# zbackup/zbackup

Measured on AMD Instinct MI355X. Metric: rolling-hash chunking GiB/s (device-resident), higher is better.
Workload: dtype u8; 1 GPU; C2: 1 x 8 GiB seeded random stream, device-resident, W=65536; stream_bytes_per_gpu=8589934592, chunk_max_size=65536, parallelism=replicas x1 (independent streams), chunk_ids=rolling hash

## Files before the change

### zbackup_amd/csrc/zc_device.h

```cpp
#pragma once

#include <hip/hip_runtime.h>
#include <stdint.h>

#include <mutex>
#include <string>

#include "../../include/zchunk.h"

struct zc_bundle_file;
struct zc_bundle_layout;
struct zc_gc_input;
struct zc_gc_output;

namespace zc {

constexpr int ZC_SPAN = 1024;
constexpr int ZC_TPB = 256;
#ifndef ZC_SCAN_TPB_CFG
#define ZC_SCAN_TPB_CFG 512
#endif
#ifndef ZC_LSPAN_CFG
#define ZC_LSPAN_CFG 4096
#endif
// ... 100 lines not shown
__host__ __device__ inline uint32_t chk_bucket(uint64_t key, uint32_t bits) {
  return (uint32_t)((key * 0x9E3779B97F4A7C15ull) >> (64 - bits));
}
__host__ __device__ inline uint32_t chk_match(uint2 v, uint32_t c) {
  const uint32_t s0 = v.x & 0xFFFFu, s1 = v.x >> 16, s2 = v.y & 0xFFFFu, s3 = v.y >> 16;
  if (s0 == c || s1 == c || s2 == c || s3 == c) return 1;
  return (s0 == 0 || s1 == 0 || s2 == 0 || s3 == 0) ? 0 : 2;
}
inline uint32_t chk_bits_for(size_t keys) {
  uint32_t b = 10;
  while (((size_t)4 << b) < 16 * keys) ++b;
  return b;
}
__host__ __device__ inline uint32_t bloom_lo(uint32_t g) {
  return (1u << (g & 31u)) | (1u << ((g >> 5) & 31u)) | (1u << ((g >> 10) & 31u));
}
__host__ __device__ inline uint32_t bloom_hi(uint32_t g) {
  return (1u << ((g >> 15) & 31u)) | (1u << ((g >> 20) & 31u)) | (1u << ((g >> 25) & 31u));
}

struct Run {
  uint64_t start, end;
};

struct Cand {
  uint64_t p;
  uint32_t ref;
  uint32_t pad;
};

enum { CNT_POOL = 0, CNT_OVERFLOW = 1, CNT_CAND = 2, CNT_RUNS = 3, CNT_FOVF = 4, CNT_ANCLESS = 5, CNT_CLASS = 6,
       CNT_PAIRS = 7, CNT_SPAIRS = 8, CNT_LAST = 9 };

hipError_t launch_scan(const uint8_t* data, uint64_t n, int32_t anchor_lo, uint64_t* blk, PoolOut po,
                       unsigned long long* counters, hipStream_t s);
hipError_t launch_scan_tiles(const uint8_t* data, uint64_t n, uint64_t tile0, uint64_t ntiles, int32_t anchor_lo,
                             uint64_t* blk, PoolOut po, unsigned long long* counters, hipStream_t s,
                             GridKeysOut gko = GridKeysOut{nullptr, nullptr, 0, 0}, hipEvent_t start = nullptr,
                             hipEvent_t stop = nullptr, uint32_t max_wgs = 0, uint32_t* tiles_per_wave = nullptr);
inline uint32_t scan_key_lshift_or_none(uint32_t W, bool& ok) {
  ok = W >= (uint32_t)ZC_LSPAN && W % ZC_LSPAN == 0 && ((64u * ZC_LSPAN) % W) == 0;
  uint32_t l = 0;
  while (ok && ((uint32_t)ZC_LSPAN << l) < W) ++l;
  return l;
}
hipError_t launch_scan_tail(const uint8_t* data, uint64_t n, int32_t anchor_lo, uint64_t* blk, PoolOut po,
                            unsigned long long* counters, hipStream_t s, hipEvent_t start = nullptr,
                            hipEvent_t stop = nullptr);

hipError_t launch_anchor_rescan(const uint8_t* data, uint64_t n, int32_t anchor_lo, const uint32_t* tiles,
                                const uint32_t* sbase, uint32_t ntiles, int pass, uint32_t* base, uint32_t* cnt,
                                uint32_t* srel, uint32_t* sg, hipStream_t s);

struct EpochIndex {
  uint64_t* start;
  uint64_t* vis;
  uint8_t* dead;
  uint64_t* key;
  uint32_t* cg;
  uint64_t* cfp;
  uint32_t* anc;
  uint32_t* cls;
  uint64_t* ckeys;
  uint32_t cbits;
  uint64_t* tab;
  uint32_t tbits;
  uint32_t* gfilt;
  uint32_t* ancless;
  unsigned long long* counters;
  uint2* pairs;
  const uint8_t* gsha;
  uint64_t n_gsha;
// ... 278 lines not shown
```

### zbackup_amd/csrc/zc_engine.cpp

```cpp
#include <hip/hip_runtime.h>
#include <stdint.h>
#include <stdio.h>
#include <stdlib.h>
#include <string.h>
#include <unistd.h>
#include <emmintrin.h>

#include <algorithm>
#include <atomic>
#include <chrono>
#include <exception>
#include <condition_variable>
#include <functional>
#include <iterator>
#include <mutex>
#include <string>
#include <thread>
#include <unordered_map>
#include <vector>

#include "../../include/zchunk.h"
#include "zc_device.h"
#include "zc_lzo_dec.h"

// ... 391 lines not shown
  uint64_t scan_out_keys = 0;
  uint32_t scan_out_tpw = 0;
  uint32_t test_scan_wgs = 0;
  HostBuf<unsigned long long> h_co_hc;
  HostBuf<Cand> h_hist_cand;
  HostBuf<uint32_t> h_cls;
  HostBuf<Run> h_runs;
  size_t nrec_done = 0;
  size_t rec_head = 0;
  mutable std::recursive_mutex mu;
  zc_stats stats{};

  LzoScratch* lzo = nullptr;
  DevBuf<uint8_t> lzo_in, lzo_out;
  AesScratch* aes = nullptr;
  GcScratch* gc = nullptr;
  MetaScratch* meta = nullptr;
  RangeScratch* range = nullptr;
  IndexScratch* index = nullptr;
  ResolveScratch* rs = nullptr;
  XzScratch* xz = nullptr;
  XzEncScratch* xzenc = nullptr;

  DevBuf<uint64_t> hm_key, hm_fp, hm_rkey;
  DevBuf<uint32_t> hm_anc, hm_g, gidx;
  DevBuf<uint64_t> blk, ftile_off;
  DevBuf<uint32_t> ftile_cnt;
  DevBuf<uint32_t> dbase, dcnt;
  DevBuf<uint32_t> prel, pg, srel, sg;
  DevBuf<uint32_t> otiles, obase;
  DevBuf<unsigned long long> counters;
  DevBuf<unsigned long long> scnt;
  bool scnt_dirty = true;
  DevBuf<uint8_t> gsha;
  HostBuf<uint2> h_pairs;
  HostBuf<uint8_t> h_gsha;
  HostBuf<uint64_t> h_hmkey;
  HostBuf<uint32_t> h_hmanc;
  DevBuf<uint64_t> c_start, c_key, c_fp, c_vis;
  DevBuf<uint32_t> c_anc, c_g;
  DevBuf<uint8_t> c_dead;
  DevBuf<uint64_t> ckeys;
  DevBuf<uint32_t> c_cls;
  DevBuf<uint64_t> tab;
  DevBuf<uint32_t> gfilt;
  DevBuf<Cand> cand;
  DevBuf<uint64_t> va, vb, dout;
  DevBuf<uint32_t> vlen;
  DevBuf<uint8_t> vok, sha_out;
  DevBuf<uint32_t> f32, fbits, fbits17;
  DevBuf<uint64_t> fwt_off;
  DevBuf<uint32_t> fwt_cnt;
  DevBuf<Run> runs;
  DevBuf<uint32_t> ancless;
  DevBuf<uint2> cpairs;
  HostBuf<unsigned long long> h_cnt;
  HostBuf<unsigned long long> h_scnt;
  HostBuf<uint64_t> h_pre;
  HostBuf<uint64_t> h_key;
  HostBuf<uint64_t> h_ra, h_rb, h_rout;
};

namespace {

struct DeviceGuard {
  int prev = -1;
// ... 224 lines not shown
    scan_keys_ = kok && !windowed_ && indexable_ && n_ >= W_ && n_ / W_ < 0xFFFFFFF0ull;
    if (scan_keys_) {
      c_.c_key.ensure(n_ / W_ + 2);
      c_.h_key.ensure(n_ / W_ + 2);
    }
    scan_setup();
  }
  void set_avail(uint64_t n) {
    n_ = n;
    c_.stats.bytes = n;
  }
  void clear_tables() {
    if (c_.tables_clean || (!c_.ckeys.p && !c_.tab.p)) return;
    if (c_.ckeys.cap % 2 || c_.tab.cap % 2 || c_.gfilt.cap % 4) return;
    HCK(launch_tables_clear(c_.ckeys.p, c_.ckeys.p ? c_.ckeys.cap : 0, c_.tab.p, c_.tab.p ? c_.tab.cap : 0,
                            c_.gfilt.p, c_.gfilt.p ? c_.gfilt.cap : 0, c_.stream));
    c_.tables_clean = true;
  }
  hipEvent_t scan_end_event() const { return (c_.flags & ZC_FLAG_TIMING) ? c_.ev1 : c_.ev_idx; }
  void scan_upto(uint64_t m, bool last = false) {
    const uint64_t t1 = std::min(m, n_) / ZC_STILE;
    if (t1 > tiles_done_) {
      hipEvent_t start = nullptr;
      if (!scan_open_) {
        if (c_.flags & ZC_FLAG_TIMING) start = c_.ev0;
        scan_open_ = true;
      }
      scnt_pending_ = true;
      const GridKeysOut gko = scan_keys_ ? GridKeysOut{c_.c_key.p, c_.h_key.p, pow257(W_), key_lshift_}
                                         : GridKeysOut{nullptr, nullptr, 0, 0};
      hipEvent_t stop = last ? scan_end_event() : nullptr;
      uint32_t tpw = 0;
      HCK(launch_scan_tiles(d_, n_, tiles_done_, t1 - tiles_done_, anchor_lo_, blk_v(), pool_out(), c_.scnt.p,
                            c_.stream, gko, start, stop, c_.test_scan_wgs, &tpw));
      scan_tpw_ = std::max(scan_tpw_, tpw);
      scan_end_recorded_ = stop != nullptr;
      tiles_done_ = t1;
    }
  }
  uint64_t scanned_end() const { return tiles_done_ * ZC_STILE; }

  void run_segment(uint64_t lim) {
    const auto t0 = Clock::now();
    scan_upto(lim);
    lim = std::min(lim, scanned_end());
    if (lim <= x0()) return;
    scan_finish();
    lim_ = lim;
    final_ = false;
    while (epoch()) {
    }
    if (!scan_checked_) {
      sync(c_);
      scan_check();
    }
    finalize_records();
    c_.stats.segments++;
    c_.stats.total_ms += ms_since(t0);
  }

  void run_final() {
    const auto t0 = Clock::now();
    if (n_ > 0) {
      const bool tail = n_ % ZC_STILE != 0;
      scan_upto(n_, !tail);
      if (tail) {
        hipEvent_t start = nullptr;
// ... 299 lines not shown
  std::vector<ACand>& acands_ = c_.res_acands;
  std::vector<ACand>& hcands_ = c_.res_hcands;

  struct FBatch {
    std::vector<uint64_t> pos, h;
    std::vector<int64_t> vref;
    std::vector<uint8_t> vok;
    std::vector<uint8_t> sha;
    std::vector<uint8_t> has_sha;
    size_t cur = 0;
  } fb_;

  struct Piece {
    size_t rec;
    uint64_t a, b;
  };
  std::vector<Piece> need_digest_;

  void scan_setup() {
    const uint64_t nwt = wave_tiles(cap_);
    if (nwt * wcap_ >= ZC_SIDE_POOL) throw ZcError{ZC_ERR_NOMEM, "stream too large for the anchor pool"};
    c_.blk.ensure((cap_ + ZC_SPAN - 1) / ZC_SPAN);
    c_.dbase.ensure(nwt);
    c_.dcnt.ensure(nwt);
    c_.prel.ensure(nwt * wcap_);
    c_.pg.ensure(nwt * wcap_);
    c_.srel.ensure(1);
    c_.sg.ensure(1);
    if (!c_.counters.p) {
      c_.counters.ensure(CNT_LAST);
      HCK(hipMemsetAsync(c_.counters.p, 0, CNT_LAST * sizeof(unsigned long long), c_.stream));
    }
    c_.h_cnt.ensure(CNT_LAST);
    c_.scnt.ensure(2);
    c_.h_scnt.ensure(CNT_LAST);
    if (c_.scnt_dirty) {
      HCK(hipMemsetAsync(c_.scnt.p, 0, 2 * sizeof(unsigned long long), c_.stream));
      c_.scnt_dirty = false;
    }
  }

  void scan_finish() {
    meta_from_scan_ = scan_open_;
    if (scan_open_) {
      if (!scan_end_recorded_) HCK(hipEventRecord(scan_end_event(), c_.stream));
      side_wait_ = scan_end_event();
      scan_end_ev_ = side_wait_;
    }
    scan_end_recorded_ = false;
    scan_checked_ = false;
  }
  void scan_counters_readback() {
    if (!scnt_pending_) return;
    scnt_pending_ = false;
    d2h(c_, c_.h_scnt.p, c_.scnt.p, 2);
    HCK(hipMemsetAsync(c_.scnt.p, 0, 2 * sizeof(unsigned long long), c_.stream));
  }

  bool scan_check() {
    if (scan_checked_) return false;
    if (scnt_pending_) {
      scan_counters_readback();
      sync(c_);
    }
    scan_checked_ = true;
    if ((c_.flags & ZC_FLAG_TIMING) && scan_open_) {
      float ms = 0;
      HCK(hipEventElapsedTime(&ms, c_.ev0, c_.ev1));
      c_.stats.scan_ms += ms;
    }
    scan_open_ = false;
    const uint64_t wt_lo = chk_wt_, wt_hi = nwt_done();
    chk_wt_ = wt_hi;
    const uint64_t found = c_.h_scnt[CNT_POOL];
    npool_ += found;
    c_.stats.anchors += found;
    if (c_.h_scnt[CNT_OVERFLOW] && wt_hi > wt_lo) {
      const uint64_t nw = wt_hi - wt_lo;
      std::vector<uint32_t> cnt(nw), tiles, sbase;
      d2h(c_, cnt.data(), dcnt_v() + wt_lo, nw);
      sync(c_);
      for (uint64_t t = 0; t < nw; ++t)
        if (cnt[t] == 0xFFFFFFFFu) tiles.push_back((uint32_t)(wt_lo + t));
      const uint32_t nt = (uint32_t)tiles.size();
      if (!nt) return false;
      c_.otiles.ensure(nt);
      c_.obase.ensure(nt);
      h2d(c_, c_.otiles.p, tiles.data(), nt);
      HCK(launch_anchor_rescan(d_, n_, anchor_lo_, c_.otiles.p, nullptr, nt, 0, dbase_v(), dcnt_v(), nullptr, nullptr,
                               c_.stream));
      std::vector<uint32_t> cnt2(nw);
      d2h(c_, cnt2.data(), dcnt_v() + wt_lo, nw);
      sync(c_);
      uint64_t total = 0;
      for (uint32_t t : tiles) {
        sbase.push_back((uint32_t)(side_used_ + total));
        total += cnt2[t - wt_lo];
      }
      if (side_used_ + total >= ZC_SIDE_POOL) throw ZcError{ZC_ERR_NOMEM, "anchor side pool too large"};
      npool_ += total;
      c_.stats.anchors += total;
      c_.srel.grow_keep(side_used_ + total, side_used_, c_.stream);
      c_.sg.grow_keep(side_used_ + total, side_used_, c_.stream);
      h2d(c_, c_.obase.p, sbase.data(), nt);
      HCK(launch_anchor_rescan(d_, n_, anchor_lo_, c_.otiles.p, c_.obase.p, nt, 1, dbase_v(), dcnt_v(), c_.srel.p,
                               c_.sg.p, c_.stream));
      side_used_ += total;
      return true;
    }
    return false;
  }
  bool scan_checked_ = true;
  bool scnt_pending_ = false;
  bool meta_from_scan_ = false;
  hipEvent_t side_wait_ = nullptr;
  hipEvent_t scan_end_ev_ = nullptr;

  bool epoch() {
    if (!scan_checked_ && c_.stats.epochs > 0) {
      sync(c_);
      scan_check();
    }
    c_.stats.epochs++;
    r_e_ = s_;
    ks_ = 0;
    grec_ = grec_valid_ = false;
    const uint64_t xs = x0();
    h_end_ = hspan_ ? std::min<uint64_t>(lim_, xs + hspan_) : lim_;
    nspec_ = (n_ >= r_e_ + 2ull * W_) ? (uint32_t)((n_ - r_e_ - 2ull * W_) / W_ + 1) : 0;
    if (h_end_ < n_) {
      const uint64_t kh = h_end_ - r_e_ >= 2ull * W_ ? (h_end_ - r_e_) / W_ - 1 : 0;
      nspec_ = (uint32_t)std::min<uint64_t>(nspec_, kh);
    }
    const uint32_t nsref = indexable_ ? nspec_ : 0;
    nref_ = nconf_ + nsref;
    dead_.assign(nref_, 0);
    ndead_ = 0;
    cls_.clear();
    acands_.clear();
    hcands_.clear();
    runs_.clear();
    fmap_.clear();
    fmemo_valid_ = false;
    fb_ = FBatch{};
    fb_next_ = kInf;
    has_f_ = false;
// ... 31 lines not shown
        c_.c_dead.ensure(nref_);
        c_.ancless.ensure(nref_);
        c_.h_key.ensure(nsref);
        if (nconf_) {
          h2d(c_, c_.c_start.p, cstart_.data(), nconf_);
          h2d(c_, c_.c_key.p, ckey_.data(), nconf_);
          h2d(c_, c_.c_fp.p, cfp_.data(), nconf_);
          h2d(c_, c_.c_anc.p, canc_.data(), nconf_);
          h2d(c_, c_.c_g.p, cg_.data(), nconf_);
          HCK(hipMemsetAsync(c_.c_vis.p, 0, nconf_ * sizeof(uint64_t), c_.stream));
          HCK(hipMemsetAsync(c_.c_dead.p, 0, nconf_, c_.stream));
        }
        tabs_new |= c_.ckeys.ensure(1u << tbits);
        if (tabs_new) {
          c_.tables_clean = false;
          c_.paths |= ZC_PATH_TABLES_REALLOCATED;
        }
        c_.c_cls.ensure(nref_);
        c_.cpairs.ensure(nref_);
        ix = EpochIndex{c_.c_start.p, c_.c_vis.p, c_.c_dead.p, c_.c_key.p,
                        c_.c_g.p,     c_.c_fp.p,  c_.c_anc.p,  c_.c_cls.p,
                        c_.ckeys.p,   tbits,      anchors ? c_.tab.p : nullptr, tbits,
                        c_.gfilt.p,   c_.ancless.p, c_.counters.p, c_.cpairs.p,
                        pre_sha_n_ ? c_.h_gsha.p : nullptr, pre_sha_n_, nsref ? c_.h_key.p : nullptr};
        ix.key_from = key_from;
        ix.tables_clean = c_.tables_clean;
        c_.tables_clean = false;
        if (key_from) c_.paths |= ZC_PATH_SCAN_KEYS;
        c_.paths |= epoch_index_fused(ix, nconf_, nsref) ? ZC_PATH_FUSED_INSERT : ZC_PATH_TABLES_CLEARED_BY_EPOCH;
        if (scnt_pending_) {
          ix.scnt = c_.scnt.p;
          ix.h_scnt = c_.h_scnt.p;
          scnt_pending_ = false;
        }
        grec_valid_ = false;
        grec_ = !windowed_ && indexable_ && nsref >= kGridRecordsMin;
        grec_ev_ = key_from == nsref && scan_end_ev_ ? scan_end_ev_ : c_.ev_grec;
        HCK(launch_epoch_index(d_, n_, blk_v(), av(), r_e_, nconf_, nsref, W_, pow257(W_), ix, c_.stream,
                               grec_ && grec_ev_ == c_.ev_grec ? c_.ev_grec : nullptr));
        dev_r_e_ = r_e_;
        dev_nconf_ = nconf_;
        dev_nspec_ = nsref;
        dev_valid_ = true;
      } else {
        HCK(hipMemsetAsync(c_.counters.p, 0, CNT_LAST * sizeof(unsigned long long), c_.stream));
        scan_counters_readback();
      }
      const uint64_t* tab = nref_ && anchors ? c_.tab.p : nullptr;
      const bool early_join = spec_ && nref_ && pre_sha_n_;
      if (early_join) HCK(launch_class_sha(nullptr, pre_sha_n_, n_, W_, ix, nref_, c_.stream));
      if (anchors)
        HCK(launch_probe(d_, av(), pwt0(), pwt1() - pwt0(), tab, tbits, c_.gfilt.p, c_.c_anc.p, c_.c_cls.p,
                         c_.c_vis.p, c_.c_dead.p, r_, h_end_, W_, ht, r_e_, nconf_, nsref, c_.cand.p, c_.cand.cap, c_.counters.p,
                         c_.stream));
      if (side_wait_) {
        HCK(hipStreamWaitEvent(c_.copy_stream, side_wait_, 0));
        side_wait_ = nullptr;
      }
      predict_tail();
      HCK(hipEventRecord(c_.ev_copy, c_.copy_stream));
      if (nsref >= kParallelRecordsMin) SpinTeam::get().arm();
      const bool first = !scan_checked_ && meta_from_scan_;
      HCK(launch_counters_out(c_.counters.p, c_.h_cnt.p, c_.stream));
      hipEvent_t batch_ev = c_.ev_batch;
      if (first && (c_.flags & ZC_FLAG_TIMING)) batch_ev = c_.ev_meta;
      HCK(hipEventRecord(batch_ev, c_.stream));
// ... 3136 lines not shown
```

### zbackup_amd/csrc/zc_kernels.hip

```cpp
#include <hip/hip_ext.h>
#include <hip/hip_runtime.h>
#include <stdint.h>

#include <algorithm>

#include "zc_device.h"

namespace zc {

namespace {

constexpr uint64_t kGolden = 0x9E3779B97F4A7C15ull;
typedef unsigned v2u32 __attribute__((ext_vector_type(2)));

#define ZC_URGENT() __builtin_amdgcn_s_setprio(3)

__host__ __device__ inline uint64_t pow257_dev(uint64_t e) {
  uint64_t r = 1, b = 257;
  while (e) {
    if (e & 1) r *= b;
    b *= b;
    e >>= 1;
  }
  return r;
// ... 278 lines not shown
    });
  }
  return tot;
}

typedef __attribute__((address_space(3))) void lds_void_t;
typedef __attribute__((address_space(1))) const void gbl_void_t;

template <int N>
__device__ __forceinline__ void wait_vmcnt() {
  static_assert(N >= 0 && N < 64, "vmcnt");
  asm volatile("s_waitcnt vmcnt(%0)" ::"n"(N) : "memory");
}

constexpr int kRounds = ZC_LSPAN / ZC_ROUND;
constexpr int kDmaRound = 64 * ZC_ROUND / 1024;
constexpr int kDigests = ZC_LSPAN / ZC_SPAN;
constexpr int kHalfRounds = kRounds / 2;
#ifndef ZC_CONTIG_PROBE_CFG
#define ZC_CONTIG_PROBE_CFG 0
#endif
constexpr bool kContigProbe = ZC_CONTIG_PROBE_CFG != 0;
constexpr uint32_t kHalfSpan = ZC_LSPAN / 2;
static_assert((kHalfRounds & (kHalfRounds - 1)) == 0 && kHalfRounds % (ZC_SPAN / ZC_ROUND) == 0, "half-span rotation");

constexpr int kPieces = ZC_ROUND / 16;
__host__ __device__ constexpr uint32_t row_swizzle(uint32_t row) { return (row / (256 / ZC_ROUND)) % kPieces; }

template <int AUX>
__device__ __forceinline__ void stage_round(const uint8_t* __restrict__ data, uint8_t* ring, uint32_t wave,
                                            const uint32_t (&lane_off)[kDmaRound], uint64_t tile, int r,
                                            uint32_t slot) {
  uint8_t* dst = ring + slot * (64 * ZC_ROUND);
  const uint64_t at = kContigProbe
                          ? tile * ZC_STILE + (uint64_t)wave * 64 * ZC_LSPAN + (uint64_t)r * 64 * ZC_ROUND
                          : tile * ZC_STILE + (uint64_t)wave * 64 * ZC_LSPAN + (uint64_t)(r % kHalfRounds) * ZC_ROUND;
  const auto rs = __builtin_amdgcn_make_buffer_rsrc((void*)(data + at), (short)0, 64 * ZC_LSPAN, 0x00020000);
  const uint32_t flip = !kContigProbe && r >= kHalfRounds ? kHalfSpan : 0u;
#pragma unroll
  for (int j = 0; j < kDmaRound; ++j)
    __builtin_amdgcn_raw_ptr_buffer_load_lds(rs, (lds_void_t*)(dst + j * 1024), 16, (int)(lane_off[j] ^ flip), 0, 0,
                                             AUX);
}

template <int N>
__device__ __forceinline__ void wait_lgkmcnt() {
  asm volatile("s_waitcnt lgkmcnt(%0)" ::"n"(N) : "memory");
}

typedef unsigned v4u32 __attribute__((ext_vector_type(4)));
__device__ __forceinline__ v4u32 lds_read16(const uint8_t* p) {
  v4u32 v;
  const uint32_t a = (uint32_t)(uintptr_t)(const __attribute__((address_space(3))) uint8_t*)p;
  asm volatile("ds_read_b128 %0, %1" : "=v"(v) : "v"(a) : "memory");
  return v;
}
__device__ __forceinline__ v4u32 global_read16(const uint8_t* p) {
  v4u32 v;
  asm volatile("global_load_dwordx4 %0, %1, off" : "=v"(v) : "v"(p) : "memory");
  return v;
}
__device__ __forceinline__ uint4 to_uint4(v4u32 v) { return make_uint4(v[0], v[1], v[2], v[3]); }
template <int N>
__device__ __forceinline__ void ties(v4u32 (&v)[N]) {
  static_assert(N == 2 || N == 4 || N == 8, "ties");
  if constexpr (N == 2) {
    asm volatile("" : "+v"(v[0]), "+v"(v[1])::"memory");
  } else if constexpr (N == 4) {
    asm volatile("" : "+v"(v[0]), "+v"(v[1]), "+v"(v[2]), "+v"(v[3])::"memory");
// ... 138 lines not shown
          const uint32_t g = dword_key(gdd, S1, S2, q);
          po.rel[base + w] = sb + t;
          po.g[base + w] = g;
          mask &= mask - 1;
          ++w;
        }
        nst += 2;
      }
    }
  }
  if (lane == 0) {
    po.base[wt] = base;
    po.cnt[wt] = over ? ZC_WT_OVERFLOW : tot;
  }
  acc_pool += over ? 0u : tot;
  acc_over += over ? 1u : 0u;
  return kDigests / 2 + __builtin_amdgcn_readfirstlane(nst) + 2 + nkey;
}

constexpr int kScanWaves = ZC_SCAN_WAVES;
#ifndef ZC_SCAN_WG_PER_CU_CFG
#define ZC_SCAN_WG_PER_CU_CFG 2
#endif
constexpr int kScanWgPerCu = ZC_SCAN_WG_PER_CU_CFG;
#ifndef ZC_SCAN_SLOTS_CFG
#define ZC_SCAN_SLOTS_CFG 1
#endif
constexpr int kScanSlots = ZC_SCAN_SLOTS_CFG;
#ifndef ZC_SCAN_PRIO_CFG
#define ZC_SCAN_PRIO_CFG 0
#endif
constexpr int kScanPrioHandoff = ZC_SCAN_PRIO_CFG;
static_assert(kScanSlots == 1 || kScanSlots == 2, "one or two ring slots");
struct ScanLds {
  uint8_t ring[kScanWaves][kScanSlots * 64 * ZC_ROUND];
  uint4 wdata[kScanWaves][ZC_WLIST];
  uint32_t wlist[kScanWaves][ZC_WLIST * 3];
};
static_assert(kScanWgPerCu * sizeof(ScanLds) <= 160 * 1024, "the scan workgroups of a CU fit its LDS");
__device__ __forceinline__ void scan_body(
    const uint8_t* __restrict__ data, uint64_t n, uint64_t wt0, uint64_t nwt, int32_t lo_thr,
    uint64_t* __restrict__ blk, PoolOut po, unsigned long long* __restrict__ counters, ScanLds& L,
    GridKeysOut gko = GridKeysOut{nullptr, nullptr, 0, 0}) {
  constexpr uint32_t kRpt = kRounds;
  constexpr uint32_t kWpt = ZC_SCAN_TPB / 64;
  const uint32_t tid = threadIdx.x, lane = tid & 63, wave = __builtin_amdgcn_readfirstlane(tid >> 6);
  const uint32_t gw = blockIdx.x * kScanWaves + wave, nw = gridDim.x * kScanWaves;
  uint8_t* myring = L.ring[wave];
  WaveList wl{L.wlist[wave], L.wdata[wave], 0};
  const uint32_t ntk = nwt > gw ? (uint32_t)((nwt - 1 - gw) / nw + 1) : 0;
  const uint32_t nR = ntk * kRpt;
  uint32_t lane_off[kDmaRound];
#pragma unroll
  for (int j = 0; j < kDmaRound; ++j) {
    const uint32_t row = j * (1024 / ZC_ROUND) + lane / kPieces;
    lane_off[j] = kContigProbe ? row * ZC_ROUND + ((lane % kPieces) ^ row_swizzle(row)) * 16
                               : row * ZC_LSPAN + (row & 1) * kHalfSpan + ((lane % kPieces) ^ row_swizzle(row)) * 16;
  }
  const uint32_t sw = row_swizzle(lane);
  const uint32_t two = pk_two();
  const uint32_t hs = (lane & 1) * kHalfRounds;
  v4u32 warm[2] = {};
  auto group = [&](uint32_t Rx) -> uint32_t { return kDmaRound + ((Rx % kRpt) % kHalfRounds == 0 ? 2u : 0u); };
  auto issue = [&](uint32_t Rx) {
    const uint32_t k = Rx / kRpt, r = Rx - k * kRpt;
    const uint64_t wt = wt0 + gw + (uint64_t)k * nw;
    stage_round<kScanDmaAux>(data, myring, (uint32_t)(wt % kWpt), lane_off, wt / kWpt, (int)r, Rx % kScanSlots);
    if (r % kHalfRounds == 0) {
      const uint64_t at = (wt << ZC_WT_SHIFT) + (uint64_t)lane * ZC_LSPAN + (uint64_t)(r ^ hs) * ZC_ROUND;
      const uint8_t* src = at >= 32 ? data + at - 32 : data + at;
      warm[0] = global_read16(src);
      warm[1] = global_read16(src + 16);
    }
  };
  uint32_t after[kScanSlots];
#pragma unroll
  for (int i = 0; i < kScanSlots; ++i) {
    after[i] = 0;
    if ((uint32_t)i < nR) {
#pragma unroll
      for (int j = 0; j < i; ++j) after[j] += group(i);
      issue(i);
    }
  }
  ScanLane s{0, 0, 0};
  uint64_t bk[kDigests];
#pragma unroll
  for (int t = 0; t < kDigests; ++t) bk[t] = 0;
  uint64_t span0 = 0;
  uint32_t last = kNoEntry;
  uint32_t acc_pool = 0, acc_over = 0;
  const uint64_t span_m = span_mul();
  const uint64_t lane_w =
      gko.key ? pow257_dev((uint64_t)ZC_LSPAN * (((1u << gko.lshift) - 1) - (lane & ((1u << gko.lshift) - 1)))) : 0;

#pragma unroll 1
  for (uint32_t R = 0; R < nR; ++R) {
    const uint32_t k = R / kRpt;
    const int r = (int)(R - k * kRpt);
    if constexpr (kScanPrioHandoff > 0) __builtin_amdgcn_s_setprio(kScanPrioHandoff);
    if (kScanSlots == 1 && r != 0) wait_vmcnt<0>();
    else wait_vmcnt_dyn(after[0]);
    const uint32_t pr = (uint32_t)r ^ hs;
    if (r == 0) {
      span0 = ((wt0 + gw + (uint64_t)k * nw) << ZC_WT_SHIFT) + (uint64_t)lane * ZC_LSPAN;
      s = ScanLane{0, 0, 0};
      wl.n = 0;
      last = kNoEntry;
    }
    if (r % kHalfRounds == 0) {
      s.glo = 0;
      ties(warm);
      if (span0 + pr * ZC_ROUND >= 64) {
        const uint32_t xs[8] = {warm[0][0], warm[0][1], warm[0][2], warm[0][3],
                                warm[1][0], warm[1][1], warm[1][2], warm[1][3]};
#pragma unroll
        for (int j = 0; j < 8; ++j) s.glo = pk_step(pk_step(s.glo, bytes01(xs[j]), two), bytes23(xs[j]), two);
      }
    }
    static_assert(kPieces % 4 == 0 && kPieces <= 16, "the round is read as 4, 8 or 16 pieces");
    constexpr int kGroups = kPieces / 4;
    v4u32 vg[kGroups][4];
#pragma unroll
    for (int g = 0; g < kGroups; ++g)
#pragma unroll
      for (int p = 0; p < 4; ++p)
        vg[g][p] = lds_read16(myring + (R % kScanSlots) * (64 * ZC_ROUND) + lane * ZC_ROUND + (((4 * g + p) ^ sw) << 4));
    wait_lgkmcnt<0>();
#pragma unroll
    for (int g = 0; g < kGroups; ++g) ties(vg[g]);
#pragma unroll
    for (int i = 0; i + 1 < kScanSlots; ++i) after[i] = after[i + 1];
    after[kScanSlots - 1] = 0;
    if (R + kScanSlots < nR) {
#pragma unroll
      for (int i = 0; i + 1 < kScanSlots; ++i) after[i] += group(R + kScanSlots);
      issue(R + kScanSlots);
    }
    if constexpr (kScanPrioHandoff > 0) __builtin_amdgcn_s_setprio(0);
#pragma unroll
    for (int g = 0; g < kGroups; ++g)
#pragma unroll
      for (int p = 0; p < 4; ++p)
        scan_piece(to_uint4(vg[g][p]), pr * ZC_ROUND + (4 * g + p) * 16, lo_thr, two, s, wl, last);
    if ((r + 1) % (ZC_SPAN / ZC_ROUND) == 0) {
      const uint64_t h = ((uint64_t)s.hhi << 32) | s.hlo;
      const uint32_t q = pr / (ZC_SPAN / ZC_ROUND);
#pragma unroll
      for (int t = 0; t < kDigests; ++t) bk[t] = q == (uint32_t)t ? h : bk[t];
      s.hlo = s.hhi = 0;
    }
    if (r == kRounds - 1) {
      const uint32_t ns =
          scan_tile_end(span0, lane, lo_thr, bk, wl, last, blk, po, acc_pool, acc_over, gko, span_m, lane_w);
#pragma unroll
      for (int i = 0; i < kScanSlots; ++i) after[i] += ns;
    }
  }
  if (lane == 0) {
    if (acc_pool) atomicAdd(&counters[CNT_POOL], (unsigned long long)acc_pool);
    if (acc_over) atomicAdd(&counters[CNT_OVERFLOW], (unsigned long long)acc_over);
  }
}

__global__ void __launch_bounds__(64 * kScanWaves, kScanWgPerCu) zc_scan_kernel(
    const uint8_t* __restrict__ data, uint64_t n, uint64_t wt0, uint64_t nwt, int32_t lo_thr,
    uint64_t* __restrict__ blk, PoolOut po, unsigned long long* __restrict__ counters, GridKeysOut gko) {
  __shared__ ScanLds lds;
  scan_body(data, n, wt0, nwt, lo_thr, blk, po, counters, lds, gko);
}
__global__ void __launch_bounds__(ZC_WT_BLOCK) zc_scan_tail_kernel(const uint8_t* __restrict__ data, uint64_t n,
                                                             uint64_t tile, int32_t lo_thr,
                                                             uint64_t* __restrict__ blk, PoolOut po,
                                                             unsigned long long* __restrict__ counters) {
  __shared__ uint32_t s_tmp[ZC_WT_BLOCK / 64];
  const uint64_t wt = tile * (ZC_SCAN_TPB / 64) + blockIdx.x;
  const uint32_t base = (uint32_t)(wt - po.wt0) * po.wcap;
  const uint32_t tot = wave_tile_block(data, n, wt, lo_thr, blk, po.rel, po.g, base, po.wcap, s_tmp);
  if (threadIdx.x == 0) {
    po.base[wt] = base;
    if (tot > po.wcap) {
      po.cnt[wt] = ZC_WT_OVERFLOW;
      atomicAdd(&counters[CNT_OVERFLOW], 1ull);
    } else {
      po.cnt[wt] = tot;
      if (tot) atomicAdd(&counters[CNT_POOL], (unsigned long long)tot);
    }
  }
}

__global__ void __launch_bounds__(ZC_WT_BLOCK) zc_anchor_rescan_kernel(const uint8_t* __restrict__ data, uint64_t n,
                                                                 int32_t lo_thr, const uint32_t* __restrict__ tiles,
                                                                 const uint32_t* __restrict__ sbase, int pass,
                                                                 uint32_t* __restrict__ dbase,
                                                                 uint32_t* __restrict__ dcnt,
                                                                 uint32_t* __restrict__ srel, uint32_t* __restrict__ sg) {
  __shared__ uint32_t s_tmp[ZC_WT_BLOCK / 64];
  const uint64_t wt = tiles[blockIdx.x];
  const uint32_t b = pass ? sbase[blockIdx.x] : 0u;
  const uint32_t tot = wave_tile_block(data, n, wt, lo_thr, nullptr, pass ? srel : nullptr, sg, b, ~0u, s_tmp);
  if (threadIdx.x == 0) {
    dcnt[wt] = tot;
// ... 92 lines not shown
}

struct FusedInsert {
  uint64_t* ckeys;
  uint32_t cbits;
  uint64_t* tab;
  uint32_t tbits;
  uint32_t* gfilt;
};
__device__ __forceinline__ void class_insert(const uint64_t* __restrict__ key, uint32_t i, uint64_t* ckeys,
                                             uint32_t cbits);
__device__ __forceinline__ void anchor_insert(uint32_t i, uint32_t g, uint64_t fp, uint64_t* tab, uint32_t tbits,
                                              uint32_t* __restrict__ gfilt);

__global__ void zc_chunk_meta_kernel(const uint8_t* __restrict__ data, uint64_t n,
                                     const uint64_t* __restrict__ blk, AnchorView av, uint64_t r_e,
                                     uint32_t nchunks, uint32_t split, uint32_t W, uint64_t pw,
                                     uint64_t* __restrict__ start, uint64_t* __restrict__ vis,
                                     uint8_t* __restrict__ dead, uint64_t* __restrict__ key,
                                     uint32_t* __restrict__ cg, uint64_t* __restrict__ cfp,
                                     uint32_t* __restrict__ anc_off, uint64_t* __restrict__ hkey, uint32_t key_from,
                                     EpochClear ec, FusedInsert fi) {
  ZC_URGENT();
  const uint64_t gt = (uint64_t)blockIdx.x * blockDim.x + threadIdx.x, gs = (uint64_t)gridDim.x * blockDim.x;
  for (uint64_t j = gt; j < ec.cwords; j += gs) ec.ckeys[j] = ~0ull;
  if (ec.tab)
    for (uint64_t j = gt; j < ec.twords; j += gs) ec.tab[j] = ~0ull;
  for (uint64_t j = gt; j < ec.gwords; j += gs) ec.gfilt[j] = 0u;
  if (gt < CNT_LAST) ec.counters[gt] = 0ull;
  if (ec.scnt && gt < 2) {
    ec.h_scnt[gt] = ec.scnt[gt];
    ec.scnt[gt] = 0ull;
  }
  if (gt < nchunks) {
    const uint32_t i = (uint32_t)gt;
    const uint64_t c = r_e + (uint64_t)i * W;
    start[i] = c;
    vis[i] = c + 2ull * W - 1;
    dead[i] = 0;
    if (i >= key_from) {
      const uint64_t k = pw + rk_acc(data, blk, c, c + W);
      key[i] = k;
      if (hkey) hkey[i] = k;
    }
    if (fi.ckeys) class_insert(key, i, fi.ckeys, fi.cbits);
  } else if (gt >= split && gt - split < nchunks) {
    const uint32_t i = (uint32_t)(gt - split);
    uint32_t off, gv;
    uint64_t f;
    first_anchor(data, av, r_e + (uint64_t)i * W, W, off, gv, f);
    anc_off[i] = off;
    cg[i] = gv;
    cfp[i] = f;
    if (fi.ckeys && fi.tab && off != ZC_NO_ANCHOR) anchor_insert(i, gv, f, fi.tab, fi.tbits, fi.gfilt);
  }
}

__global__ void zc_ref_meta_kernel(const uint8_t* __restrict__ data, const uint64_t* __restrict__ blk, AnchorView av,
                                   const uint64_t* __restrict__ starts, uint32_t cnt, uint32_t split, uint32_t W,
                                   uint64_t pw, uint64_t* __restrict__ key, uint32_t* __restrict__ anc_off,
                                   uint32_t* __restrict__ cg, uint64_t* __restrict__ cfp) {
  ZC_URGENT();
  const uint64_t gt = (uint64_t)blockIdx.x * blockDim.x + threadIdx.x;
  if (gt < cnt) {
    const uint64_t c = starts[gt];
    key[gt] = pw + rk_acc(data, blk, c, c + W);
// ... 1576 lines not shown
  for (; i < nw + 1; i += stride) {
    uint64_t z = seed + (i + 1) * kGolden;
    z = (z ^ (z >> 30)) * 0xBF58476D1CE4E5B9ull;
    z = (z ^ (z >> 27)) * 0x94D049BB133111EBull;
    z ^= z >> 31;
    if (i < nw) {
      ((uint64_t*)d)[i] = z;
    } else {
      for (uint64_t k = nw * 8; k < n; ++k) d[k] = (uint8_t)(z >> (8 * (k - nw * 8)));
    }
  }
}

inline unsigned blocks_for(uint64_t items, unsigned per) { return (unsigned)((items + per - 1) / per); }

}

uint64_t pow257(uint64_t e) { return pow257_dev(e); }

static int cu_count() {
  static int cus = 0;
  if (!cus) {
    int dev = 0;
    if (hipGetDevice(&dev) != hipSuccess ||
        hipDeviceGetAttribute(&cus, hipDeviceAttributeMultiprocessorCount, dev) != hipSuccess || cus <= 0)
      cus = 256;
  }
  return cus;
}

hipError_t launch_scan_tiles(const uint8_t* data, uint64_t n, uint64_t tile0, uint64_t ntiles, int32_t anchor_lo,
                             uint64_t* blk, PoolOut po, unsigned long long* counters, hipStream_t s,
                             GridKeysOut gko, hipEvent_t start, hipEvent_t stop, uint32_t max_wgs,
                             uint32_t* tiles_per_wave) {
  if (tiles_per_wave) *tiles_per_wave = 0;
  if (!ntiles) return hipSuccess;
  if (gko.key && (!gko.hkey || ((uint64_t)ZC_LSPAN << gko.lshift) > (1ull << ZC_WT_SHIFT))) return hipErrorInvalidValue;
  const uint64_t wt0 = tile0 * (ZC_SCAN_TPB / 64), nwt = ntiles * (ZC_SCAN_TPB / 64);
  unsigned grid = (unsigned)std::min<uint64_t>((nwt + kScanWaves - 1) / kScanWaves,
                                               (uint64_t)cu_count() * kScanWgPerCu);
  if (max_wgs && max_wgs < grid) grid = max_wgs;
  if (tiles_per_wave) *tiles_per_wave = (uint32_t)((nwt - 1) / ((uint64_t)grid * kScanWaves) + 1);
  if (start || stop)
    hipExtLaunchKernelGGL(zc_scan_kernel, dim3(grid), dim3(64 * kScanWaves), 0, s, start, stop, 0, data, n, wt0, nwt,
                          anchor_lo, blk, po, counters, gko);
  else
    hipLaunchKernelGGL(zc_scan_kernel, dim3(grid), dim3(64 * kScanWaves), 0, s, data, n, wt0, nwt, anchor_lo, blk,
                       po, counters, gko);
  return hipGetLastError();
}

hipError_t launch_scan_tail(const uint8_t* data, uint64_t n, int32_t anchor_lo, uint64_t* blk, PoolOut po,
                            unsigned long long* counters, hipStream_t s, hipEvent_t start, hipEvent_t stop) {
  if (n % ZC_STILE) {
    if (start || stop)
      hipExtLaunchKernelGGL(zc_scan_tail_kernel, dim3(ZC_SCAN_TPB / 64), dim3(ZC_WT_BLOCK), 0, s, start, stop, 0, data,
                            n, (uint64_t)(n / ZC_STILE), anchor_lo, blk, po, counters);
    else
      hipLaunchKernelGGL(zc_scan_tail_kernel, dim3(ZC_SCAN_TPB / 64), dim3(ZC_WT_BLOCK), 0, s, data, n, n / ZC_STILE,
                         anchor_lo, blk, po, counters);
  }
  return hipGetLastError();
}

hipError_t launch_scan(const uint8_t* data, uint64_t n, int32_t anchor_lo, uint64_t* blk, PoolOut po,
                       unsigned long long* counters, hipStream_t s) {
  hipError_t e = launch_scan_tiles(data, n, 0, n / ZC_STILE, anchor_lo, blk, po, counters, s);
  if (e != hipSuccess) return e;
  return launch_scan_tail(data, n, anchor_lo, blk, po, counters, s);
}

hipError_t launch_anchor_rescan(const uint8_t* data, uint64_t n, int32_t anchor_lo, const uint32_t* tiles,
                                const uint32_t* sbase, uint32_t ntiles, int pass, uint32_t* base, uint32_t* cnt,
                                uint32_t* srel, uint32_t* sg, hipStream_t s) {
  if (!ntiles) return hipSuccess;
  hipLaunchKernelGGL(zc_anchor_rescan_kernel, dim3(ntiles), dim3(ZC_WT_BLOCK), 0, s, data, n, anchor_lo, tiles, sbase,
                     pass, base, cnt, srel, sg);
  return hipGetLastError();
}





hipError_t launch_epoch_index(const uint8_t* data, uint64_t n, const uint64_t* blk, AnchorView av, uint64_t r_e,
                              uint32_t nconf, uint32_t nsref, uint32_t W, uint64_t pw, const EpochIndex& ix,
                              hipStream_t s, hipEvent_t after_meta) {
  const uint32_t nref = nconf + nsref;
  const bool fused = epoch_index_fused(ix, nconf, nsref);
  const EpochClear ec{ix.ckeys, nref && !fused ? 1u << ix.cbits : 0u, ix.tab,
                      ix.tab && !fused ? 2ull << ix.tbits : 0ull, ix.gfilt, ix.tab && !fused ? kGFiltWords : 0u,
                      ix.counters, ix.scnt, ix.h_scnt};
  const FusedInsert fi{fused ? ix.ckeys : nullptr, ix.cbits, ix.tab, ix.tbits, ix.gfilt};
  const uint64_t words = (uint64_t)ec.cwords + ec.twords + ec.gwords;
  const uint32_t split = (uint32_t)(blocks_for(nsref, 128) * 128);
  const uint64_t threads =
      std::max<uint64_t>({(uint64_t)split + nsref, std::min<uint64_t>(words / 4, 1u << 20), CNT_LAST});
  hipLaunchKernelGGL(zc_chunk_meta_kernel, dim3(blocks_for(threads, 128)), dim3(128), 0, s, data, n, blk, av, r_e,
                     nsref, split, W, pw, ix.start + nconf, ix.vis + nconf, ix.dead + nconf, ix.key + nconf,
                     ix.cg + nconf, ix.cfp + nconf, ix.anc + nconf, ix.hkey, ix.key_from, ec, fi);
// ... 347 lines not shown
```

Baseline: 5332 GiB/s.

## Claim scan wave-tiles dynamically via atomic counter instead of static striding

Replaces the static round-robin assignment of wave-tiles to waves in the scan kernel with a dynamic work queue: each wave issues an atomic claim one tile ahead, mid-tile, and picks up the next tile when the claim is in range. The aim is to balance work across waves and CUs so slow or late-starting waves no longer set the tail of the kernel. The host tracks a cumulative claim base and checks that the claims add up after readback. It also makes the staging address wave-uniform via readfirstlane and skips the warm-up reads on even lanes at mid-tile, carrying the rolling hash over instead. In exchange the scan pays one atomic per tile and must use a single ring slot. An optional timestamp probe is included but off by default.

```diff
diff --git a/zbackup_amd/csrc/zc_device.h b/zbackup_amd/csrc/zc_device.h
--- a/zbackup_amd/csrc/zc_device.h
+++ b/zbackup_amd/csrc/zc_device.h
@@ -156,12 +156,18 @@
 enum { CNT_POOL = 0, CNT_OVERFLOW = 1, CNT_CAND = 2, CNT_RUNS = 3, CNT_FOVF = 4, CNT_ANCLESS = 5, CNT_CLASS = 6,
        CNT_PAIRS = 7, CNT_SPAIRS = 8, CNT_LAST = 9 };
 
+struct ScanClaim {
+  uint32_t* counter;
+  uint32_t base;
+};
+
 hipError_t launch_scan(const uint8_t* data, uint64_t n, int32_t anchor_lo, uint64_t* blk, PoolOut po,
-                       unsigned long long* counters, hipStream_t s);
+                       unsigned long long* counters, hipStream_t s, ScanClaim claim = ScanClaim{nullptr, 0});
 hipError_t launch_scan_tiles(const uint8_t* data, uint64_t n, uint64_t tile0, uint64_t ntiles, int32_t anchor_lo,
                              uint64_t* blk, PoolOut po, unsigned long long* counters, hipStream_t s,
                              GridKeysOut gko = GridKeysOut{nullptr, nullptr, 0, 0}, hipEvent_t start = nullptr,
-                             hipEvent_t stop = nullptr, uint32_t max_wgs = 0, uint32_t* tiles_per_wave = nullptr);
+                             hipEvent_t stop = nullptr, uint32_t max_wgs = 0, uint32_t* tiles_per_wave = nullptr,
+                             ScanClaim claim = ScanClaim{nullptr, 0});
 inline uint32_t scan_key_lshift_or_none(uint32_t W, bool& ok) {
   ok = W >= (uint32_t)ZC_LSPAN && W % ZC_LSPAN == 0 && ((64u * ZC_LSPAN) % W) == 0;
   uint32_t l = 0;
diff --git a/zbackup_amd/csrc/zc_engine.cpp b/zbackup_amd/csrc/zc_engine.cpp
--- a/zbackup_amd/csrc/zc_engine.cpp
+++ b/zbackup_amd/csrc/zc_engine.cpp
@@ -447,6 +447,7 @@
   DevBuf<unsigned long long> counters;
   DevBuf<unsigned long long> scnt;
   bool scnt_dirty = true;
+  uint32_t claim_base = 0;
   DevBuf<uint8_t> gsha;
   HostBuf<uint2> h_pairs;
   HostBuf<uint8_t> h_gsha;
@@ -737,7 +738,9 @@
       hipEvent_t stop = last ? scan_end_event() : nullptr;
       uint32_t tpw = 0;
       HCK(launch_scan_tiles(d_, n_, tiles_done_, t1 - tiles_done_, anchor_lo_, blk_v(), pool_out(), c_.scnt.p,
-                            c_.stream, gko, start, stop, c_.test_scan_wgs, &tpw));
+                            c_.stream, gko, start, stop, c_.test_scan_wgs, &tpw,
+                            ScanClaim{(uint32_t*)(c_.scnt.p + 2), c_.claim_base}));
+      c_.claim_base += (uint32_t)((t1 - tiles_done_) * (ZC_SCAN_TPB / 64));
       scan_tpw_ = std::max(scan_tpw_, tpw);
       scan_end_recorded_ = stop != nullptr;
       tiles_done_ = t1;
@@ -1103,10 +1106,11 @@
       HCK(hipMemsetAsync(c_.counters.p, 0, CNT_LAST * sizeof(unsigned long long), c_.stream));
     }
     c_.h_cnt.ensure(CNT_LAST);
-    c_.scnt.ensure(2);
+    c_.scnt.ensure(3);
     c_.h_scnt.ensure(CNT_LAST);
     if (c_.scnt_dirty) {
-      HCK(hipMemsetAsync(c_.scnt.p, 0, 2 * sizeof(unsigned long long), c_.stream));
+      HCK(hipMemsetAsync(c_.scnt.p, 0, 3 * sizeof(unsigned long long), c_.stream));
+      c_.claim_base = 0;
       c_.scnt_dirty = false;
     }
   }
@@ -1124,7 +1128,9 @@
   void scan_counters_readback() {
     if (!scnt_pending_) return;
     scnt_pending_ = false;
-    d2h(c_, c_.h_scnt.p, c_.scnt.p, 2);
+    claim_expect_ = c_.claim_base;
+    claim_handed_ = true;
+    d2h(c_, c_.h_scnt.p, c_.scnt.p, 3);
     HCK(hipMemsetAsync(c_.scnt.p, 0, 2 * sizeof(unsigned long long), c_.stream));
   }
 
@@ -1143,6 +1149,11 @@
     scan_open_ = false;
     const uint64_t wt_lo = chk_wt_, wt_hi = nwt_done();
     chk_wt_ = wt_hi;
+    if (claim_handed_ && (uint32_t)c_.h_scnt[2] != claim_expect_) {
+      c_.scnt_dirty = true;
+      throw ZcError{ZC_ERR_STATE, "internal error: the scan's wave-tile claims do not add up"};
+    }
+    claim_handed_ = false;
     const uint64_t found = c_.h_scnt[CNT_POOL];
     npool_ += found;
     c_.stats.anchors += found;
@@ -1183,6 +1194,8 @@
   }
   bool scan_checked_ = true;
   bool scnt_pending_ = false;
+  uint32_t claim_expect_ = 0;
+  bool claim_handed_ = false;
   bool meta_from_scan_ = false;
   hipEvent_t side_wait_ = nullptr;
   hipEvent_t scan_end_ev_ = nullptr;
@@ -1280,6 +1293,8 @@
           ix.scnt = c_.scnt.p;
           ix.h_scnt = c_.h_scnt.p;
           scnt_pending_ = false;
+          claim_expect_ = c_.claim_base;
+          claim_handed_ = true;
         }
         grec_valid_ = false;
         grec_ = !windowed_ && indexable_ && nsref >= kGridRecordsMin;
diff --git a/zbackup_amd/csrc/zc_kernels.hip b/zbackup_amd/csrc/zc_kernels.hip
--- a/zbackup_amd/csrc/zc_kernels.hip
+++ b/zbackup_amd/csrc/zc_kernels.hip
@@ -334,9 +334,12 @@
                                             const uint32_t (&lane_off)[kDmaRound], uint64_t tile, int r,
                                             uint32_t slot) {
   uint8_t* dst = ring + slot * (64 * ZC_ROUND);
-  const uint64_t at = kContigProbe
-                          ? tile * ZC_STILE + (uint64_t)wave * 64 * ZC_LSPAN + (uint64_t)r * 64 * ZC_ROUND
-                          : tile * ZC_STILE + (uint64_t)wave * 64 * ZC_LSPAN + (uint64_t)(r % kHalfRounds) * ZC_ROUND;
+  const uint64_t at_u = kContigProbe
+                            ? tile * ZC_STILE + (uint64_t)wave * 64 * ZC_LSPAN + (uint64_t)r * 64 * ZC_ROUND
+                            : tile * ZC_STILE + (uint64_t)wave * 64 * ZC_LSPAN +
+                                  (uint64_t)((uint32_t)r & (uint32_t)(kHalfRounds - 1)) * ZC_ROUND;
+  const uint64_t at = ((uint64_t)(uint32_t)__builtin_amdgcn_readfirstlane((uint32_t)(at_u >> 32)) << 32) |
+                      (uint64_t)(uint32_t)__builtin_amdgcn_readfirstlane((uint32_t)at_u);
   const auto rs = __builtin_amdgcn_make_buffer_rsrc((void*)(data + at), (short)0, 64 * ZC_LSPAN, 0x00020000);
   const uint32_t flip = !kContigProbe && r >= kHalfRounds ? kHalfSpan : 0u;
 #pragma unroll
@@ -541,6 +544,28 @@
 #endif
 constexpr int kScanPrioHandoff = ZC_SCAN_PRIO_CFG;
 static_assert(kScanSlots == 1 || kScanSlots == 2, "one or two ring slots");
+#ifndef ZC_SCAN_CLAIM_CFG
+#define ZC_SCAN_CLAIM_CFG 1
+#endif
+constexpr bool kScanClaim = ZC_SCAN_CLAIM_CFG != 0;
+static_assert(!kScanClaim || kScanSlots == 1, "the claim is prefetched one tile ahead: one ring slot");
+constexpr int kClaimRound = 8;
+#ifndef ZC_SCAN_ROLL_CFG
+#define ZC_SCAN_ROLL_CFG 1
+#endif
+constexpr bool kScanRoll = ZC_SCAN_ROLL_CFG != 0;
+#ifndef ZC_SCAN_STAMP_CFG
+#define ZC_SCAN_STAMP_CFG 0
+#endif
+#if ZC_SCAN_STAMP_CFG
+__device__ uint32_t* g_scan_stamp;
+#endif
+__device__ __forceinline__ uint32_t claim_issue(uint32_t* counter) {
+  uint32_t v;
+  const uint32_t one = 1;
+  asm volatile("global_atomic_add %0, %1, %2, off sc0" : "=v"(v) : "v"(counter), "v"(one) : "memory");
+  return v;
+}
 struct ScanLds {
   uint8_t ring[kScanWaves][kScanSlots * 64 * ZC_ROUND];
   uint4 wdata[kScanWaves][ZC_WLIST];
@@ -550,15 +575,24 @@
 __device__ __forceinline__ void scan_body(
     const uint8_t* __restrict__ data, uint64_t n, uint64_t wt0, uint64_t nwt, int32_t lo_thr,
     uint64_t* __restrict__ blk, PoolOut po, unsigned long long* __restrict__ counters, ScanLds& L,
-    GridKeysOut gko = GridKeysOut{nullptr, nullptr, 0, 0}) {
+    GridKeysOut gko = GridKeysOut{nullptr, nullptr, 0, 0}, ScanClaim claim = ScanClaim{nullptr, 0}) {
   constexpr uint32_t kRpt = kRounds;
   constexpr uint32_t kWpt = ZC_SCAN_TPB / 64;
   const uint32_t tid = threadIdx.x, lane = tid & 63, wave = __builtin_amdgcn_readfirstlane(tid >> 6);
   const uint32_t gw = blockIdx.x * kScanWaves + wave, nw = gridDim.x * kScanWaves;
   uint8_t* myring = L.ring[wave];
   WaveList wl{L.wlist[wave], L.wdata[wave], 0};
-  const uint32_t ntk = nwt > gw ? (uint32_t)((nwt - 1 - gw) / nw + 1) : 0;
-  const uint32_t nR = ntk * kRpt;
+#if ZC_SCAN_STAMP_CFG
+  const uint64_t stamp_t0 = wall_clock64();
+#endif
+  const uint32_t ntk = kScanClaim ? (nwt > gw ? 1u : 0u) : nwt > gw ? (uint32_t)((nwt - 1 - gw) / nw + 1) : 0;
+  uint32_t nR = ntk * kRpt;
+  uint64_t wt_cur = wt0 + gw, wt_nxt = 0;
+  uint32_t kc = 0;
+  uint32_t claim_v = 0;
+  auto tile_of = [&](uint32_t k) -> uint64_t {
+    return kScanClaim ? (k == kc ? wt_cur : wt_nxt) : wt0 + gw + (uint64_t)k * nw;
+  };
   uint32_t lane_off[kDmaRound];
 #pragma unroll
   for (int j = 0; j < kDmaRound; ++j) {
@@ -573,13 +607,15 @@
   auto group = [&](uint32_t Rx) -> uint32_t { return kDmaRound + ((Rx % kRpt) % kHalfRounds == 0 ? 2u : 0u); };
   auto issue = [&](uint32_t Rx) {
     const uint32_t k = Rx / kRpt, r = Rx - k * kRpt;
-    const uint64_t wt = wt0 + gw + (uint64_t)k * nw;
+    const uint64_t wt = tile_of(k);
     stage_round<kScanDmaAux>(data, myring, (uint32_t)(wt % kWpt), lane_off, wt / kWpt, (int)r, Rx % kScanSlots);
     if (r % kHalfRounds == 0) {
       const uint64_t at = (wt << ZC_WT_SHIFT) + (uint64_t)lane * ZC_LSPAN + (uint64_t)(r ^ hs) * ZC_ROUND;
       const uint8_t* src = at >= 32 ? data + at - 32 : data + at;
-      warm[0] = global_read16(src);
-      warm[1] = global_read16(src + 16);
+      if (!kScanRoll || r == 0 || (lane & 1)) {
+        warm[0] = global_read16(src);
+        warm[1] = global_read16(src + 16);
+      }
     }
   };
   uint32_t after[kScanSlots];
@@ -612,19 +648,32 @@
     else wait_vmcnt_dyn(after[0]);
     const uint32_t pr = (uint32_t)r ^ hs;
     if (r == 0) {
-      span0 = ((wt0 + gw + (uint64_t)k * nw) << ZC_WT_SHIFT) + (uint64_t)lane * ZC_LSPAN;
+      if (kScanClaim && k != kc) {
+        wt_cur = wt_nxt;
+        kc = k;
+      }
+      span0 = (tile_of(k) << ZC_WT_SHIFT) + (uint64_t)lane * ZC_LSPAN;
       s = ScanLane{0, 0, 0};
       wl.n = 0;
       last = kNoEntry;
     }
     if (r % kHalfRounds == 0) {
-      s.glo = 0;
       ties(warm);
+      uint32_t g = 0;
       if (span0 + pr * ZC_ROUND >= 64) {
         const uint32_t xs[8] = {warm[0][0], warm[0][1], warm[0][2], warm[0][3],
                                 warm[1][0], warm[1][1], warm[1][2], warm[1][3]};
 #pragma unroll
-        for (int j = 0; j < 8; ++j) s.glo = pk_step(pk_step(s.glo, bytes01(xs[j]), two), bytes23(xs[j]), two);
+        for (int j = 0; j < 8; ++j) g = pk_step(pk_step(g, bytes01(xs[j]), two), bytes23(xs[j]), two);
+      }
+      s.glo = kScanRoll && r != 0 && !(lane & 1) ? s.glo : g;
+    }
+    if (kScanClaim && r == kClaimRound + 1) {
+      asm volatile("" : "+v"(claim_v)::"memory");
+      const uint32_t c = __builtin_amdgcn_readfirstlane(claim_v) - claim.base;
+      if ((uint64_t)c + nw < nwt) {
+        wt_nxt = wt0 + nw + c;
+        nR += kRpt;
       }
     }
     static_assert(kPieces % 4 == 0 && kPieces <= 16, "the round is read as 4, 8 or 16 pieces");
@@ -646,6 +695,7 @@
       for (int i = 0; i + 1 < kScanSlots; ++i) after[i] += group(R + kScanSlots);
       issue(R + kScanSlots);
     }
+    if (kScanClaim && r == kClaimRound && lane == 0) claim_v = claim_issue(claim.counter);
     if constexpr (kScanPrioHandoff > 0) __builtin_amdgcn_s_setprio(0);
 #pragma unroll
     for (int g = 0; g < kGroups; ++g)
@@ -670,13 +720,23 @@
     if (acc_pool) atomicAdd(&counters[CNT_POOL], (unsigned long long)acc_pool);
     if (acc_over) atomicAdd(&counters[CNT_OVERFLOW], (unsigned long long)acc_over);
   }
+#if ZC_SCAN_STAMP_CFG
+  if (lane == 0 && g_scan_stamp) {
+    const uint64_t t1 = wall_clock64();
+    const uint32_t hw = __builtin_amdgcn_s_getreg(4 | (31 << 11)), xcc = __builtin_amdgcn_s_getreg(20 | (31 << 11));
+    uint4* o = (uint4*)(g_scan_stamp + 8 * gw);
+    o[0] = make_uint4((uint32_t)stamp_t0, (uint32_t)(stamp_t0 >> 32), (uint32_t)t1, (uint32_t)(t1 >> 32));
+    o[1] = make_uint4(hw, xcc, nR / kRpt, gw);
+  }
+#endif
 }
 
 __global__ void __launch_bounds__(64 * kScanWaves, kScanWgPerCu) zc_scan_kernel(
     const uint8_t* __restrict__ data, uint64_t n, uint64_t wt0, uint64_t nwt, int32_t lo_thr,
-    uint64_t* __restrict__ blk, PoolOut po, unsigned long long* __restrict__ counters, GridKeysOut gko) {
+    uint64_t* __restrict__ blk, PoolOut po, unsigned long long* __restrict__ counters, GridKeysOut gko,
+    ScanClaim claim) {
   __shared__ ScanLds lds;
-  scan_body(data, n, wt0, nwt, lo_thr, blk, po, counters, lds, gko);
+  scan_body(data, n, wt0, nwt, lo_thr, blk, po, counters, lds, gko, claim);
 }
 __global__ void __launch_bounds__(ZC_WT_BLOCK) zc_scan_tail_kernel(const uint8_t* __restrict__ data, uint64_t n,
                                                              uint64_t tile, int32_t lo_thr,
@@ -835,6 +895,7 @@
     ec.h_scnt[gt] = ec.scnt[gt];
     ec.scnt[gt] = 0ull;
   }
+  if (ec.scnt && gt == 2) ec.h_scnt[2] = ec.scnt[2];
   if (gt < nchunks) {
     const uint32_t i = (uint32_t)gt;
     const uint64_t c = r_e + (uint64_t)i * W;
@@ -2477,9 +2538,10 @@
 hipError_t launch_scan_tiles(const uint8_t* data, uint64_t n, uint64_t tile0, uint64_t ntiles, int32_t anchor_lo,
                              uint64_t* blk, PoolOut po, unsigned long long* counters, hipStream_t s,
                              GridKeysOut gko, hipEvent_t start, hipEvent_t stop, uint32_t max_wgs,
-                             uint32_t* tiles_per_wave) {
+                             uint32_t* tiles_per_wave, ScanClaim claim) {
   if (tiles_per_wave) *tiles_per_wave = 0;
   if (!ntiles) return hipSuccess;
+  if (kScanClaim && (!claim.counter || ntiles * (ZC_SCAN_TPB / 64) > 0xFFFFFFFFull)) return hipErrorInvalidValue;
   if (gko.key && (!gko.hkey || ((uint64_t)ZC_LSPAN << gko.lshift) > (1ull << ZC_WT_SHIFT))) return hipErrorInvalidValue;
   const uint64_t wt0 = tile0 * (ZC_SCAN_TPB / 64), nwt = ntiles * (ZC_SCAN_TPB / 64);
   unsigned grid = (unsigned)std::min<uint64_t>((nwt + kScanWaves - 1) / kScanWaves,
@@ -2488,10 +2550,10 @@
   if (tiles_per_wave) *tiles_per_wave = (uint32_t)((nwt - 1) / ((uint64_t)grid * kScanWaves) + 1);
   if (start || stop)
     hipExtLaunchKernelGGL(zc_scan_kernel, dim3(grid), dim3(64 * kScanWaves), 0, s, start, stop, 0, data, n, wt0, nwt,
-                          anchor_lo, blk, po, counters, gko);
+                          anchor_lo, blk, po, counters, gko, claim);
   else
     hipLaunchKernelGGL(zc_scan_kernel, dim3(grid), dim3(64 * kScanWaves), 0, s, data, n, wt0, nwt, anchor_lo, blk,
-                       po, counters, gko);
+                       po, counters, gko, claim);
   return hipGetLastError();
 }
 
@@ -2509,8 +2571,9 @@
 }
 
 hipError_t launch_scan(const uint8_t* data, uint64_t n, int32_t anchor_lo, uint64_t* blk, PoolOut po,
-                       unsigned long long* counters, hipStream_t s) {
-  hipError_t e = launch_scan_tiles(data, n, 0, n / ZC_STILE, anchor_lo, blk, po, counters, s);
+                       unsigned long long* counters, hipStream_t s, ScanClaim claim) {
+  hipError_t e = launch_scan_tiles(data, n, 0, n / ZC_STILE, anchor_lo, blk, po, counters, s,
+                                   GridKeysOut{nullptr, nullptr, 0, 0}, nullptr, nullptr, 0, nullptr, claim);
   if (e != hipSuccess) return e;
   return launch_scan_tail(data, n, anchor_lo, blk, po, counters, s);
 }
```

Measured after the change: 5600 GiB/s (median of 6 runs). +5.0%, better.
